# jltsiren/bwt-merge

Measured on AMD Instinct MI355X. Metric: merged Gbases/sec (input1+input2), bit-exact native BWT; value = inputs and result resident in HBM, host_to_host_value = SURVEY 8(d)'s T (page-locked host to page-locked host), higher is better.
Workload: dtype u64

## Files before the change

bwt-merge_amd/csrc/api/context.hip.h:

```cpp
#pragma once


namespace
{

thread_local std::string g_error;

int fail(int code, const char* fmt, ...)
{
  char buf[512];
  va_list ap; va_start(ap, fmt); vsnprintf(buf, sizeof(buf), fmt, ap); va_end(ap);
  g_error = buf;
  return code;
}

inline u64 div_up(u64 a, u64 b) { return (a + b - 1) / b; }

}


struct bwtm_context
{
  int device = -1;
  hipStream_t stream = nullptr;
// ... 3 lines not shown
  std::atomic<long long> live_handles{0};

  bool profiling = false;
  std::string profile_only;
  bool profile_open = false;
  struct Pending { const char* name; hipEvent_t start, stop; };
  std::vector<Pending> pending;
  std::map<std::string, std::pair<double, uint64_t>> totals;
  std::vector<const char*> order;

  std::multimap<u64, void*> free_blocks;
  u64 cached_bytes = 0, held_bytes = 0, peak_bytes = 0;
  struct VBlock { u64 bytes = 0; std::vector<hipMemGenericAllocationHandle_t> chunks; hipEvent_t released = nullptr; };
  bool vmm = false;
  std::vector<hipMemGenericAllocationHandle_t> free_chunks;
  std::map<void*, VBlock> vblocks;
  u64 device_total = 0;
  u64 va_fallbacks = 0;

  void* stream_stage[4] = {nullptr, nullptr, nullptr, nullptr};
  u64 stream_stage_cap[4] = {0, 0, 0, 0};
  u64* host_scratch = nullptr;
  u64 scan1_tiles = 0, pull_scan1_tiles = 0;
  u64 step_forms[3] = {0, 0, 0};
  u64 transcode_forms[16] = {};
};

namespace
{

struct Tuning
{
  long long search_algo = 0;
  long long frontier_unfused = 0;
  long long l1_cap = 0;
  long long emit_path = 0;
  long long round_emits = 1ll << 33;
  long long emit_budget = 0;
  long long frontier_epoch = 512;
  long long eager_cum_budget = 16ll << 30;
  long long upload_chunk = 256ll << 20;
  long long download_chunk = 128ll << 20;
  long long range_ratio = 8;
#ifdef BWTM_EXPERIMENTAL
  long long search_view = 0;
#endif
  long long frontier_stage_out = 1;
  long long frontier_rel = 1;
  long long frontier_parts = 0;
  long long part_capacity = 0;
  long long recs_uniform = 0;
  long long recs_window = 0;
  long long stream_samples_query = 0;
  long long stream_upload = 0;
  long long extract_batch = 1ll << 20;
  long long locate_batch = 1ll << 20;
  long long overlap_batch = 1ll << 20;
  long long mem_batch = 1ll << 20;
  long long approx_batch = 1ll << 16;
  long long correct_batch = 1ll << 20;
  long long ingest_verify = 0;
#ifdef BWTM_DIAGNOSTICS
  long long walk_emit = 0;
  long long walk_blocks = 0;
  long long walk_kernel = 0;
  long long walk_ablate = 0;
// ... 24 lines not shown
void pool_trim(bwtm_context* c);
void stream_stage_free(bwtm_context* c)
{
  for(int k = 0; k < 4; k++) { if(c->stream_stage[k]) { (void)hipHostFree(c->stream_stage[k]); } c->stream_stage[k] = nullptr; c->stream_stage_cap[k] = 0; }
}
void apply_env_tuning();

int context_setup(bwtm_context* c, int device)
{
  int count = 0;
  hipError_t e = hipGetDeviceCount(&count);
  if(e != hipSuccess || count <= 0) { return fail(BWTM_ENODEV, "no HIP device available (%s)", hipGetErrorString(e)); }
  if(device < 0 || device >= count) { return fail(BWTM_EINVAL, "device %d out of range (%d devices)", device, count); }
  HIP_TRY(hipSetDevice(device));
  apply_env_tuning();
  c->device = device;
  HIP_TRY(hipStreamCreateWithFlags(&c->stream, hipStreamNonBlocking));
  HIP_TRY(hipStreamCreateWithFlags(&c->copy_stream, hipStreamNonBlocking));
  HIP_TRY(hipHostMalloc((void**)&c->host_scratch, 128 * sizeof(u64), hipHostMallocDefault));
  vmm_setup(c);
  {
    hipDeviceProp_t prop;
    HIP_TRY(hipGetDeviceProperties(&prop, device));
    int per_cu_scan = 0, per_cu_pull = 0;
    HIP_TRY(hipOccupancyMaxActiveBlocksPerMultiprocessor(&per_cu_scan, (const void*)k_frontier_scan1, BLOCK_THREADS, 0));
    HIP_TRY(hipOccupancyMaxActiveBlocksPerMultiprocessor(&per_cu_pull, (const void*)k_pull_scan1, BLOCK_THREADS, 0));
    c->scan1_tiles = std::min<u64>(FRONTIER_SCAN1_TILES, (u64)std::max(per_cu_scan, 0) * (u64)std::max(prop.multiProcessorCount, 0));
    c->pull_scan1_tiles = std::min<u64>(FRONTIER_SCAN1_TILES, (u64)std::max(per_cu_pull, 0) * (u64)std::max(prop.multiProcessorCount, 0));
  }
  HIP_TRY(hipFuncSetAttribute((const void*)k_part_scatter_sorted, hipFuncAttributeMaxDynamicSharedMemorySize, 96 * 1024));
  HIP_TRY(hipFuncSetAttribute((const void*)k_lf_walk_binned<true>, hipFuncAttributeMaxDynamicSharedMemorySize, 40 * 1024));
#ifdef BWTM_DIAGNOSTICS
  HIP_TRY(hipFuncSetAttribute((const void*)k_lf_walk_lds<true>, hipFuncAttributeMaxDynamicSharedMemorySize, 122 * 1024));
  HIP_TRY(hipFuncSetAttribute((const void*)k_lf_walk_lds<false>, hipFuncAttributeMaxDynamicSharedMemorySize, 82 * 1024));
#endif
  return BWTM_OK;
}

void context_teardown(bwtm_context* c)
{
  if(c->device < 0) { return; }
  (void)hipSetDevice(c->device);
  if(c->stream) { (void)hipStreamSynchronize(c->stream); }
  if(c->copy_stream) { (void)hipStreamSynchronize(c->copy_stream); }
  for(auto& p : c->pending) { (void)hipEventDestroy(p.start); (void)hipEventDestroy(p.stop); }
  c->pending.clear();
  pool_trim(c);
  stream_stage_free(c);
  if(c->host_scratch) { (void)hipHostFree(c->host_scratch); }
  if(c->stream) { (void)hipStreamDestroy(c->stream); }
  if(c->copy_stream) { (void)hipStreamDestroy(c->copy_stream); }
// ... 441 lines not shown
  {
    fail(BWTM_EINVAL, "bwtm_context_destroy: %lld handles of the context are still alive; context not destroyed", context->live_handles.load());
    return;
  }
  context_teardown(context);
  delete context;
}

extern "C" const char* bwtm_last_error(void) { return g_error.c_str(); }

namespace
{
int tune_set(const char* key, long long value)
{
  std::string k(key);
  if(k == "search_algo") { g_tune.search_algo = value; }
  else if(k == "frontier_unfused") { g_tune.frontier_unfused = value; }
  else if(k == "l1_cap") { g_tune.l1_cap = value; }
  else if(k == "emit_path") { g_tune.emit_path = value; }
  else if(k == "round_emits") { g_tune.round_emits = (value > 0 ? value : 1); }
  else if(k == "emit_budget") { g_tune.emit_budget = (value > 0 ? value : 0); }
  else if(k == "frontier_epoch") { g_tune.frontier_epoch = (value > 0 ? value : 512); }
  else if(k == "range_ratio") { g_tune.range_ratio = (value >= 0 ? value : 8); }
#ifdef BWTM_EXPERIMENTAL
  else if(k == "search_view") { g_tune.search_view = (value >= 0 && value <= 2 ? value : 0); }
#endif
  else if(k == "frontier_stage_out") { g_tune.frontier_stage_out = (value != 0); }
  else if(k == "frontier_rel") { g_tune.frontier_rel = (value >= 0 && value <= 2 ? value : 1); }
  else if(k == "frontier_parts") { g_tune.frontier_parts = (value > 0 ? value : 0); }
  else if(k == "stream_samples_query") { g_tune.stream_samples_query = (value != 0); }
  else if(k == "stream_upload") { g_tune.stream_upload = (value != 0); }
  else if(k == "ingest_verify") { g_tune.ingest_verify = (value != 0); }
  else if(k == "extract_batch") { g_tune.extract_batch = (value > 0 ? value : (1ll << 20)); }
  else if(k == "locate_batch") { g_tune.locate_batch = (value > 0 ? std::min<long long>(value, 1ll << 28) : (1ll << 20)); }
  else if(k == "overlap_batch") { g_tune.overlap_batch = (value > 0 ? std::min<long long>(value, 1ll << 28) : (1ll << 20)); }
  else if(k == "mem_batch") { g_tune.mem_batch = (value > 0 ? std::min<long long>(value, 1ll << 28) : (1ll << 20)); }
  else if(k == "approx_batch") { g_tune.approx_batch = (value > 0 ? std::min<long long>(value, 1ll << 28) : (1ll << 16)); }
  else if(k == "correct_batch") { g_tune.correct_batch = (value > 0 ? std::min<long long>(value, 1ll << 28) : (1ll << 20)); }
  else if(k == "part_capacity") { g_tune.part_capacity = value; }
  else if(k == "recs_uniform") { g_tune.recs_uniform = (value > 0 ? 1 : (value < 0 ? -1 : 0)); }
  else if(k == "recs_window") { g_tune.recs_window = (value == 8192 || value == 16384 || value == 32768 ? value : 0); }
  else if(k == "eager_cum_budget") { g_tune.eager_cum_budget = (value > 0 ? value : (16ll << 30)); }
  else if(k == "upload_chunk") { g_tune.upload_chunk = (value > 0 ? value : (256ll << 20)); }
  else if(k == "download_chunk") { g_tune.download_chunk = (value > 0 ? value : (128ll << 20)); }
#ifdef BWTM_DIAGNOSTICS
  else if(k == "walk_emit") { g_tune.walk_emit = value; }
// ... 167 lines not shown
```

bwt-merge_amd/csrc/api/partition.hip.h:

```cpp
#pragma once

extern "C" int bwtm_fslice_set_cuts(bwtm_fslice* fs, const uint64_t* r_cuts, int parts)
{
  if(!fs || !r_cuts || parts < 1 || parts > BWTM_X_MAX_PARTS) { return fail(BWTM_EINVAL, "bwtm_fslice_set_cuts: bad argument (at most %d parts)", BWTM_X_MAX_PARTS); }
  for(int k = 0; k < parts; k++) { if(r_cuts[k] > r_cuts[k + 1] && k + 1 < parts) { return fail(BWTM_EINVAL, "bwtm_fslice_set_cuts: cuts must not decrease"); } }
  if(r_cuts[0] != 0) { return fail(BWTM_EINVAL, "bwtm_fslice_set_cuts: the first cut is 0"); }
  ENTER(fs->ctx);
  if((u32)(5 * parts) > fs->max_pieces) { return fail(BWTM_EINVAL, "bwtm_fslice_set_cuts: more parts than the slice was created for"); }
  fs->ncuts = (u32)parts + 1;
  TRY(fs->cuts.alloc(fs->ncuts * sizeof(u64))); TRY(fs->below.alloc(5ull * fs->ncuts * sizeof(u64), true));
  if(!fs->host_below) { HIP_TRY(hipHostMalloc((void**)&fs->host_below, 5ull * (BWTM_X_MAX_PARTS + 1) * sizeof(u64), hipHostMallocDefault)); }
  if(!fs->dense_lo)
  {
    const u64 fcap = fs->nbl * FR_BLOCK;
    TRY(fslice_export_alloc(fs, fs->dense_lo, fcap));
    if(fs->wide) { TRY(fslice_export_alloc(fs, fs->dense_hi, fcap)); }
    TRY(fs->dense_pieces.alloc((u64)fs->max_pieces * sizeof(DensePiece)));
    HIP_TRY(hipHostMalloc((void**)&fs->host_dense_pieces, (u64)fs->max_pieces * sizeof(DensePiece), hipHostMallocDefault));
  }
  std::memset(fs->host_below, 0, 5ull * (BWTM_X_MAX_PARTS + 1) * sizeof(u64));
  u64 host_cuts[BWTM_X_MAX_PARTS + 1];
  for(int k = 0; k <= parts; k++) { host_cuts[k] = (k == parts ? ~0ull : r_cuts[k]); }
  HIP_TRY(hipMemcpyAsync(fs->cuts.p, host_cuts, fs->ncuts * sizeof(u64), hipMemcpyHostToDevice, CTX.stream));
  HIP_TRY(hipStreamSynchronize(CTX.stream));
// ... 213 lines not shown

extern "C" int bwtm_fslice_nodes_expand(bwtm_fslice* fs)
{
  if(!fs) { return fail(BWTM_EINVAL, "bwtm_fslice_nodes_expand: null argument"); }
  ENTER(fs->ctx);
  if(!fs->node_sp[0]) { return fail(BWTM_EINVAL, "bwtm_fslice_nodes_expand: call bwtm_fslice_nodes_begin first"); }
  const u64 N = fs->nodes;
  u64 alive = 0;
  DevBuf offsets;
  if(N > 0)
  {
    TRY(offsets.alloc((N + 1) * sizeof(u64)));
    HIP_TRY(hipMemcpyAsync(offsets.p, fs->node_cnt[0], N * sizeof(u64), hipMemcpyDeviceToDevice, CTX.stream));
    HIP_TRY(hipMemsetAsync(offsets.as<u64>() + N, 0, sizeof(u64), CTX.stream));
    TRY(device_scan<0>(offsets.as<u64>(), offsets.as<u64>(), N + 1));
    TRY(fetch_u64(offsets.as<u64>() + N, 0));
    HIP_TRY(hipStreamSynchronize(CTX.stream));
    alive = CTX.host_scratch[0];
  }
  if(alive > fs->cap) { return fail(BWTM_EINVAL, "bwtm_fslice_nodes_expand: the nodes stand for %llu sequences, capacity %llu", (unsigned long long)alive, (unsigned long long)fs->cap); }
  fs->nb_out = std::max<u64>(1, div_up(alive, (u64)FR_BLOCK));
  if(N > 0)
  {
    LAUNCH("range_expand", k_range_expand, div_up(N, BLOCK_THREADS), BLOCK_THREADS, (const u64*)fs->node_sp[0], (const u64*)fs->node_r[0], (const u64*)fs->node_cnt[0],
      offsets.as<const u64>(), N, fs->lo_out, fs->hi_out, fs->node_pieces.as<RangePiece>(), fs->node_npieces.as<u32>(), fs->node_piece_cap);
    LAUNCH("range_expand_pieces", k_range_expand_pieces, 2048, BLOCK_THREADS, fs->node_pieces.as<const RangePiece>(), fs->node_npieces.as<const u32>(), fs->node_piece_cap, fs->lo_out, fs->hi_out);
    HIP_TRY(hipMemsetAsync(fs->node_npieces.p, 0, sizeof(u32), CTX.stream));
  }
  LAUNCH("frontier_init", k_frontier_init_tables, div_up(5 * fs->nb_out + 1, BLOCK_THREADS), BLOCK_THREADS, fs->seg_len_out.as<u64>(), fs->seg_phys_out, fs->nb_out, alive);
  fs->nodes = 0;
  TRY(fslice_scan_outputs(fs));
  return BWTM_OK;
}

extern "C" int bwtm_x_index_upload_window(const uint8_t* data, uint64_t nbytes, uint64_t first_position, const uint64_t counts_before[6],
  uint64_t bases, uint64_t sequences, const uint64_t C[7], bwtm_index** out)
{
  ENTER(nullptr);
  return index_upload_window(data, nbytes, first_position, counts_before, bases, sequences, C, false, out);
}

extern "C" int bwtm_x_ra_create_range(const bwtm_index* a, const bwtm_index* b, uint64_t pos_first, uint64_t pos_last, bwtm_ra** out)
{
  return bwtm_ra_create_range(a, b, pos_first, pos_last, out);
}

extern "C" int bwtm_x_ra_or_range(bwtm_ra* dst, const bwtm_ra* src, uint64_t pos_first, uint64_t pos_last)
// ... 52 lines not shown
```

bwt-merge_amd/csrc/api/pmerge.hip.h:

```cpp
#pragma once


namespace
{

int index_upload_window(const u8* data, u64 nbytes, u64 first_position, const u64 counts_before[6], u64 bases, u64 sequences, const u64 C[7], bool on_device, bwtm_index** out)
{
  if(!out || (nbytes > 0 && !data) || !counts_before || !C) { return fail(BWTM_EINVAL, "bwtm_index_upload_window: null argument"); }
  if(nbytes == 0 && bases != 0) { return fail(BWTM_EINVAL, "bwtm_index_upload_window: no bytes of an index of %llu positions", (unsigned long long)bases); }
  u64 before = 0; for(int c = 0; c < 6; c++) { before += counts_before[c]; }
  if(before != first_position || first_position > bases) { return fail(BWTM_EINVAL, "bwtm_index_upload_window: the counts before the bytes add up to %llu, their first position is %llu", (unsigned long long)before, (unsigned long long)first_position); }
  if(on_device && ((uintptr_t)data & 15) != 0) { return fail(BWTM_EINVAL, "bwtm_index_upload_window: a device share must be 16-byte aligned (whole 64-byte blocks of a 16-byte aligned stream)"); }
  bwtm_index* x = new bwtm_index();
  x->ctx = t_ctx; x->nbytes = nbytes;
  auto body = [&]() -> int
  {
    const bool borrow = on_device && nbytes > 0;
    if(borrow) { x->borrowed = data; }
    else { TRY(alloc_native(x->data, nbytes)); }
    int rc = upload_queue(x, (borrow || nbytes == 0) ? nullptr : data);
    if(rc == BWTM_OK) { rc = upload_scan(x, 0); }
    hipError_t e1 = hipStreamSynchronize(CTX.copy_stream), e2 = hipStreamSynchronize(CTX.stream);
    if(rc != BWTM_OK) { return rc; }
    if(e1 != hipSuccess || e2 != hipSuccess) { return fail(BWTM_ENODEV, "upload failed: %s", hipGetErrorString(e1 != hipSuccess ? e1 : e2)); }
// ... 543 lines not shown
    }
    lvl++;
  }
  S.P->info.node_levels = lvl;
  done = (level_nodes == 0);
  nb_out = 1;
  if(done) { return BWTM_OK; }
  TURN(S.G);
  u64 alive = 0;
  if(N > 0)
  {
    TRY(offsets.alloc((N + 1) * 8));
    HIP_TRY(hipMemcpyAsync(offsets.p, cnt.p, N * 8, hipMemcpyDeviceToDevice, CTX.stream));
    HIP_TRY(hipMemsetAsync(offsets.as<u64>() + N, 0, 8, CTX.stream));
    TRY(device_scan<0>(offsets.as<u64>(), offsets.as<u64>(), N + 1));
    TRY(fetch_u64(offsets.as<u64>() + N, 0));
    HIP_TRY(hipStreamSynchronize(CTX.stream));
    alive = CTX.host_scratch[0];
  }
  if(alive > S.cap) { return fail(BWTM_ENOMEM, "bwtm_part_search: the nodes of part %d stand for %llu sequences, capacity %llu", S.g, (unsigned long long)alive, (unsigned long long)S.cap); }
  nb_out = std::max<u64>(1, div_up(alive, (u64)FR_BLOCK));
  if(N > 0)
  {
    LAUNCH("range_expand", k_range_expand, div_up(N, BLOCK_THREADS), BLOCK_THREADS, sp.as<const u64>(), r.as<const u64>(), cnt.as<const u64>(), offsets.as<const u64>(), N,
      S.mine<uint2>(S.lay.lo[0]), (S.wide ? S.mine<unsigned short>(S.lay.hi[0]) : nullptr), pieces.as<RangePiece>(), npieces.as<u32>(), piece_cap);
    LAUNCH("range_expand_pieces", k_range_expand_pieces, 2048, BLOCK_THREADS, pieces.as<const RangePiece>(), npieces.as<const u32>(), piece_cap,
      S.mine<uint2>(S.lay.lo[0]), (S.wide ? S.mine<unsigned short>(S.lay.hi[0]) : nullptr));
  }
  LAUNCH("frontier_init", k_frontier_init_tables, div_up(5 * nb_out + 1, BLOCK_THREADS), BLOCK_THREADS, S.mine<u64>(S.lay.seg_len[0]), S.mine<u64>(S.lay.seg_phys[0]), nb_out, alive);
  return BWTM_OK;
}

int part_search(PartSearch& S)
{
  bwtm_part* P = S.P;
  const u64 m = P->mb;
  const u64 root_first = std::min<u64>(P->cut_b[S.g], m), root_last = std::min<u64>(P->cut_b[S.g + 1], m);
  int owners = 0;
  for(int h = 0; h < S.parts; h++) { if(std::min<u64>(P->cut_b[h + 1], m) > std::min<u64>(P->cut_b[h], m)) { owners++; } }
  const u64 limit = (g_tune.range_ratio > 0 ? std::max<u64>(1, std::min<u64>(m / (u64)g_tune.range_ratio, 1ull << 24)) : 0);
  const bool use_nodes = (limit >= 1 && owners == 1);
  TRY(search_setup(S, use_nodes));
  u64 nb_out = 1;
  int par = 0;
  if(use_nodes)
  {
    bool done = false;
// ... 238 lines not shown
```

bwt-merge_amd/csrc/api/search.hip.h:

```cpp
#pragma once

struct bwtm_ra
{
  bwtm_context* ctx = nullptr;
  bwtm_ra() : ctx(t_ctx) { if(ctx) { ctx->live_handles++; } }
  ~bwtm_ra() { if(ctx) { ctx->live_handles--; } }
  bwtm_ra(const bwtm_ra&) = delete; bwtm_ra& operator=(const bwtm_ra&) = delete;
  u64 na = 0, nb = 0, n_out = 0;
  u64 nrecs_out = 0, nchunks = 0;
  DevBuf owned_bits;
  void* bits_ptr = nullptr;
  template<class T> T* bits_as() const { return (T*)bits_ptr; }
  DevBuf chunk_base;
  bool finalized = false;
  u64 values = 0;
  bool ranged = false;
  u64 range_first = 0, range_last = 0;
  DevBuf range_rel;
  DevBuf super_boff;
  bool windowed = false;
  u64 win_word_first = 0, win_words = 0;
};

#define WHOLE_RA(ra, who) if((ra)->windowed) { return fail(BWTM_EINVAL, who ": a window of a rank array (bwtm_ra_create_range) only serves the merge over partitioned records and the output-range entry points"); }
// ... 171 lines not shown
    {
      LAUNCH_LDS("lf_walk", k_lf_walk_binned<false>, blocks, WB_THREADS, 0, a->view(), b->view(), r_first, r_count, sink, (u32)a->nsup, (u32)b->nsup);
    }

    TRY(partition_level2(l1, gcount, cap, nsub, 1, ra));
  }
  return BWTM_OK;
}

int frontier_flush(bwtm_ra* ra, DevBuf& emit16, u64 emit_cap, DevBuf& emit_base, DevBuf& bound, u64 ntiles, u64 nsteps, u64 tile_first = 0)
{
  if(nsteps == 0) { return BWTM_OK; }
  const u64 nsegs = div_up(ntiles, BOUND_SEG);
  DevBuf segmin; TRY(segmin.alloc(nsteps * nsegs * sizeof(u32)));
  LAUNCH2D("bound_seg_min", k_bound_seg_min, nsegs, nsteps, BLOCK_THREADS, bound.as<const u32>(), ntiles, nsegs, segmin.as<u32>());
  LAUNCH2D("bound_suffix_min", k_bound_suffix_min, nsegs, nsteps, BLOCK_THREADS, bound.as<u32>(), ntiles, nsegs, segmin.as<const u32>(), emit_base.as<const u64>());
  LAUNCH("tile_build", k_tile_build_frontier, ntiles, BLOCK_THREADS, emit16.as<const unsigned short>(), emit_base.as<const u64>(), emit_cap, bound.as<const u32>(),
    ntiles, nsteps, ra->bits_as<u64>() + (tile_first << (TILE_SHIFT - 6)), ra->nchunks * CHUNK_WORDS - (tile_first << (TILE_SHIFT - 6)));
  return BWTM_OK;
}

struct RangeLevels
{
  DevBuf sp[2], r[2], cnt[2], flags, pieces, npieces;
  u64 N = 0, alive = 0, levels = 0;
  u32 piece_cap = 0;
  int cur = 0;
  void release() { for(int k = 0; k < 2; k++) { sp[k].release(); r[k].release(); cnt[k].release(); } flags.release(); pieces.release(); npieces.release(); }
};

int range_phase(const bwtm_index* a, const bwtm_index* b, u64 seq_first, u64 count, bwtm_ra* ra, u64 limit, RangeLevels& L)
{
  const u64 cap = std::min<u64>(5 * limit, count) + 1;
  for(int k = 0; k < 2; k++) { TRY(L.sp[k].alloc(cap * sizeof(u64))); TRY(L.r[k].alloc(cap * sizeof(u64))); TRY(L.cnt[k].alloc(cap * sizeof(u64))); }
  TRY(L.flags.alloc((5 * limit + 1) * sizeof(u64)));
  L.piece_cap = (u32)std::min<u64>(count / 16 + 1024, 1ull << 24);
  TRY(L.pieces.alloc((u64)L.piece_cap * sizeof(RangePiece)));
  TRY(L.npieces.alloc(sizeof(u32), true));
  LAUNCH("range_init", k_range_init, 1, BLOCK_THREADS, L.sp[0].as<u64>(), L.r[0].as<u64>(), L.cnt[0].as<u64>(), seq_first, count, a->m);
  L.N = 1; L.alive = count; L.cur = 0; L.levels = 0;
  while(L.N > 0 && L.N <= limit)
  {
    const int c = L.cur;
    const u64 N = L.N, grid = div_up(N, BLOCK_THREADS);
    LAUNCH("range_step", k_range_step<false>, grid, BLOCK_THREADS, a->view(), b->view(), L.sp[c].as<const u64>(), L.r[c].as<const u64>(), L.cnt[c].as<const u64>(), N,
      L.flags.as<u64>(), (const u64*)nullptr, (u64*)nullptr, (u64*)nullptr, (u64*)nullptr, ra->bits_as<u32>(), L.pieces.as<RangePiece>(), L.npieces.as<u32>(), L.piece_cap);
    LAUNCH("range_emit", k_range_emit, 2048, BLOCK_THREADS, L.pieces.as<const RangePiece>(), L.npieces.as<const u32>(), L.piece_cap, ra->bits_as<u32>());
    HIP_TRY(hipMemsetAsync(L.npieces.p, 0, sizeof(u32), CTX.stream));
    TRY(device_scan<0>(L.flags.as<u64>(), L.flags.as<u64>(), 5 * N + 1));
    LAUNCH("range_children", k_range_step<true>, grid, BLOCK_THREADS, a->view(), b->view(), L.sp[c].as<const u64>(), L.r[c].as<const u64>(), L.cnt[c].as<const u64>(), N,
      (u64*)nullptr, L.flags.as<const u64>(), L.sp[1 - c].as<u64>(), L.r[1 - c].as<u64>(), L.cnt[1 - c].as<u64>(), (u32*)nullptr, (RangePiece*)nullptr, (u32*)nullptr, 0u);
    TRY(fetch_u64(L.flags.as<u64>() + 5 * N, 0));
    HIP_TRY(hipStreamSynchronize(CTX.stream));
    L.N = CTX.host_scratch[0];
    L.cur = 1 - c; L.levels++;
  }
  return BWTM_OK;
}

int range_alive(RangeLevels& L, DevBuf& offsets)
{
  TRY(offsets.alloc((L.N + 1) * sizeof(u64)));
  HIP_TRY(hipMemcpyAsync(offsets.p, L.cnt[L.cur].p, L.N * sizeof(u64), hipMemcpyDeviceToDevice, CTX.stream));
  HIP_TRY(hipMemsetAsync(offsets.as<u64>() + L.N, 0, sizeof(u64), CTX.stream));
  TRY(device_scan<0>(offsets.as<u64>(), offsets.as<u64>(), L.N + 1));
  TRY(fetch_u64(offsets.as<u64>() + L.N, 0));
  HIP_TRY(hipStreamSynchronize(CTX.stream));
  L.alive = CTX.host_scratch[0];
  return BWTM_OK;
}

int range_expand(RangeLevels& L, const DevBuf& offsets, uint2* lo, unsigned short* hi)
{
  const int c = L.cur;
  LAUNCH("range_expand", k_range_expand, div_up(L.N, BLOCK_THREADS), BLOCK_THREADS, L.sp[c].as<const u64>(), L.r[c].as<const u64>(), L.cnt[c].as<const u64>(),
    offsets.as<const u64>(), L.N, lo, hi, L.pieces.as<RangePiece>(), L.npieces.as<u32>(), L.piece_cap);
  LAUNCH("range_expand_pieces", k_range_expand_pieces, 2048, BLOCK_THREADS, L.pieces.as<const RangePiece>(), L.npieces.as<const u32>(), L.piece_cap, lo, hi);
  return BWTM_OK;
}

constexpr u64 FRONTIER_MIN_SEQUENCES = 1ull << 21;

int search_frontier(const bwtm_index* a, const bwtm_index* b, u64 seq_first, u64 count, bwtm_ra* ra)
{
  if(a->n >= (1ull << 40) || b->n >= (1ull << 40) || count >= (1ull << 32)) { return search_partitioned(a, b, seq_first, count, ra); }
  RangeLevels levels;
  DevBuf node_offsets;
  const bool node_phase = (g_tune.range_ratio > 0);
  if(node_phase)
  {
    const u64 limit = std::max<u64>(1, std::min<u64>(count / (u64)g_tune.range_ratio, 1ull << 24));
    TRY(range_phase(a, b, seq_first, count, ra, limit, levels));
    if(levels.N == 0) { return BWTM_OK; }
    TRY(range_alive(levels, node_offsets));
    count = levels.alive;
    if(count == 0) { return BWTM_OK; }
  }
  const u64 ntiles = div_up(ra->n_out + 1, 1ull << TILE_SHIFT);
// ... 363 lines not shown
```

bwt-merge_amd/csrc/kernels/search_range.hip.h:

```cpp
#pragma once

constexpr u32 RANGE_INLINE_WORDS = 4;
constexpr u32 RANGE_PIECE_WORDS = 2048;
constexpr u32 RANGE_EXPAND_INLINE = 48;
constexpr u32 RANGE_EXPAND_PIECE = 1024;

struct RangePiece { u64 first; u64 count; u64 aux; u64 dst; };

__device__ inline void range_set_bits(u32* bits, u64 p0, u64 p1)
{
  for(u64 w = p0 >> 5; w <= ((p1 - 1) >> 5); w++)
  {
    const u64 lo = (w << 5 > p0 ? w << 5 : p0), hi = (((w + 1) << 5) < p1 ? (w + 1) << 5 : p1);
    const u32 n = (u32)(hi - lo), sh = (u32)(lo & 31);
    const u32 mask = (n == 32 ? 0xFFFFFFFFu : ((1u << n) - 1u) << sh);
    atomicOr(bits + w, mask);
  }
}

__global__ void __launch_bounds__(BLOCK_THREADS) k_range_init(u64* sp, u64* r, u64* cnt, u64 seq_first, u64 count, u64 m_a)
{
  if(blockIdx.x == 0 && threadIdx.x == 0) { sp[0] = seq_first; r[0] = m_a; cnt[0] = count; }
}

template<bool WRITE>
__global__ void __launch_bounds__(BLOCK_THREADS) k_range_step(IndexView A, IndexView B, const u64* sp, const u64* r, const u64* cnt, u64 N,
  u64* flags, const u64* prefix, u64* sp_next, u64* r_next, u64* cnt_next, u32* bits, RangePiece* pieces, u32* npieces, u32 piece_cap)
{
  const u64 u = (u64)blockIdx.x * BLOCK_THREADS + threadIdx.x;
  if(u >= N) { return; }
  const u64 s = sp[u], k = cnt[u], rr = r[u];
  u64 rs[6], re[6];
  index_ranks(B, s, rs);
  index_ranks(B, s + k, re);
  if(!WRITE)
  {
#pragma unroll
    for(u32 c = 1; c < 6; c++) { flags[(u64)(c - 1) * N + u] = (re[c] > rs[c] ? 1 : 0); }
    if(u == 0) { flags[5 * N] = 0; }
    const u64 p0 = s + rr, p1 = p0 + k;
    if(((p1 - 1) >> 5) - (p0 >> 5) < RANGE_INLINE_WORDS) { range_set_bits(bits, p0, p1); }
    else
    {
      const u64 per = (u64)RANGE_PIECE_WORDS * 32;
      const u64 first_cut = ((p0 / per) + 1) * per;
      const u32 n = (u32)(p1 <= first_cut ? 1 : 1 + (p1 - first_cut + per - 1) / per);
      const u32 at = atomicAdd(npieces, n);
      u64 b = p0;
      for(u32 q = 0; q < n; q++)
      {
        u64 e = (b / per + 1) * per; if(e > p1) { e = p1; }
        if(at + q < piece_cap) { RangePiece pc; pc.first = b; pc.count = e - b; pc.aux = 0; pc.dst = 0; pieces[at + q] = pc; }
        else { range_set_bits(bits, b, e); }
        b = e;
      }
    }
  }
  else
  {
    u64 ra[6];
    index_ranks(A, rr, ra);
#pragma unroll
    for(u32 c = 1; c < 6; c++)
    {
      if(re[c] > rs[c])
      {
        const u64 d = prefix[(u64)(c - 1) * N + u];
        sp_next[d] = B.C[c] + rs[c];
        cnt_next[d] = re[c] - rs[c];
        r_next[d] = A.C[c] + ra[c];
      }
    }
  }
}

__global__ void __launch_bounds__(BLOCK_THREADS) k_range_emit(const RangePiece* pieces, const u32* npieces, u32 piece_cap, u32* bits)
{
  u32 n = *npieces; if(n > piece_cap) { n = piece_cap; }
  for(u32 q = blockIdx.x; q < n; q += gridDim.x)
  {
    const u64 p0 = pieces[q].first, p1 = p0 + pieces[q].count;
    const u64 w0 = p0 >> 5, w1 = (p1 - 1) >> 5;
    for(u64 w = w0 + threadIdx.x; w <= w1; w += BLOCK_THREADS)
    {
      const u64 lo = (w << 5 > p0 ? w << 5 : p0), hi = (((w + 1) << 5) < p1 ? (w + 1) << 5 : p1);
      const u32 nb = (u32)(hi - lo), sh = (u32)(lo & 31);
      atomicOr(bits + w, (nb == 32 ? 0xFFFFFFFFu : ((1u << nb) - 1u) << sh));
    }
  }
}

__device__ inline void range_store_element(uint2* lo, unsigned short* hi, u64 g, u64 i, u64 r)
{
  lo[g] = make_uint2((u32)i, (u32)r);
  if(hi) { hi[g] = (unsigned short)(((i >> 32) & 0xFF) | (((r >> 32) & 0xFF) << 8)); }
}

__global__ void __launch_bounds__(BLOCK_THREADS) k_range_expand(const u64* sp, const u64* r, const u64* cnt, const u64* offset, u64 N,
  uint2* lo, unsigned short* hi, RangePiece* pieces, u32* npieces, u32 piece_cap)
{
  const u64 u = (u64)blockIdx.x * BLOCK_THREADS + threadIdx.x;
  if(u >= N) { return; }
  const u64 s = sp[u], k = cnt[u], rr = r[u], g0 = offset[u];
  if(k <= RANGE_EXPAND_INLINE) { for(u64 j = 0; j < k; j++) { range_store_element(lo, hi, g0 + j, s + j, rr); } return; }
  const u32 n = (u32)((k + RANGE_EXPAND_PIECE - 1) / RANGE_EXPAND_PIECE);
  const u32 at = atomicAdd(npieces, n);
  for(u32 q = 0; q < n; q++)
  {
    const u64 b = (u64)q * RANGE_EXPAND_PIECE;
    const u64 c = (k - b < (u64)RANGE_EXPAND_PIECE ? k - b : (u64)RANGE_EXPAND_PIECE);
    if(at + q < piece_cap) { RangePiece pc; pc.first = s + b; pc.count = c; pc.aux = rr; pc.dst = g0 + b; pieces[at + q] = pc; }
    else { for(u64 j = 0; j < c; j++) { range_store_element(lo, hi, g0 + b + j, s + b + j, rr); } }
  }
}

__global__ void __launch_bounds__(BLOCK_THREADS) k_range_expand_pieces(const RangePiece* pieces, const u32* npieces, u32 piece_cap, uint2* lo, unsigned short* hi)
{
  u32 n = *npieces; if(n > piece_cap) { n = piece_cap; }
  for(u32 q = blockIdx.x; q < n; q += gridDim.x)
  {
    const RangePiece pc = pieces[q];
    for(u64 j = threadIdx.x; j < pc.count; j += BLOCK_THREADS) { range_store_element(lo, hi, pc.dst + j, pc.first + j, pc.aux); }
  }
}

__global__ void __launch_bounds__(BLOCK_THREADS) k_frontier_init_tables(u64* seg_len, u64* seg_phys, u64 nb_max, u64 count)
// ... 12 lines not shown
```

Measured before the change: 93.29.

## Fuse range-search level into single-pass kernel with decoupled look-back scan

Replaces the per-level two-kernel flow (flag pass, device scan, children pass) with one persistent kernel that computes child counts, publishes tile aggregates and inclusive prefixes, and scatters children in one pass using decoupled look-back. Children are written into five class-strided segments, so a RangeForm mapping is threaded through the counts and expand kernels. This removes two kernel launches and a full device scan per level, plus the flag buffer traffic. In exchange it adds spin-polling with a timeout that falls back to a compaction and a two-pass redo, tag-based tile reuse, and dependence on forward progress across co-resident blocks.

Result: no change. 94.20 (median of 6 runs) (+1.0%).

```diff
diff --git a/bwt-merge_amd/csrc/api/context.hip.h b/bwt-merge_amd/csrc/api/context.hip.h
--- a/bwt-merge_amd/csrc/api/context.hip.h
+++ b/bwt-merge_amd/csrc/api/context.hip.h
@@ -49,6 +49,7 @@
   u64 stream_stage_cap[4] = {0, 0, 0, 0};
   u64* host_scratch = nullptr;
   u64 scan1_tiles = 0, pull_scan1_tiles = 0;
+  u64 range_grid = 0;
   u64 step_forms[3] = {0, 0, 0};
   u64 transcode_forms[16] = {};
 };
@@ -69,6 +70,10 @@
   long long upload_chunk = 256ll << 20;
   long long download_chunk = 128ll << 20;
   long long range_ratio = 8;
+  long long range_single_pass = 1;
+  long long range_grid = 0;
+  long long range_piece_cap = 0;
+  long long range_expire_level = 0;
 #ifdef BWTM_EXPERIMENTAL
   long long search_view = 0;
 #endif
@@ -139,11 +144,13 @@
   {
     hipDeviceProp_t prop;
     HIP_TRY(hipGetDeviceProperties(&prop, device));
-    int per_cu_scan = 0, per_cu_pull = 0;
+    int per_cu_scan = 0, per_cu_pull = 0, per_cu_range = 0;
     HIP_TRY(hipOccupancyMaxActiveBlocksPerMultiprocessor(&per_cu_scan, (const void*)k_frontier_scan1, BLOCK_THREADS, 0));
     HIP_TRY(hipOccupancyMaxActiveBlocksPerMultiprocessor(&per_cu_pull, (const void*)k_pull_scan1, BLOCK_THREADS, 0));
     c->scan1_tiles = std::min<u64>(FRONTIER_SCAN1_TILES, (u64)std::max(per_cu_scan, 0) * (u64)std::max(prop.multiProcessorCount, 0));
     c->pull_scan1_tiles = std::min<u64>(FRONTIER_SCAN1_TILES, (u64)std::max(per_cu_pull, 0) * (u64)std::max(prop.multiProcessorCount, 0));
+    HIP_TRY(hipOccupancyMaxActiveBlocksPerMultiprocessor(&per_cu_range, (const void*)k_range_level, BLOCK_THREADS, 0));
+    c->range_grid = (u64)std::max(per_cu_range, 0) * (u64)std::max(prop.multiProcessorCount, 0);
   }
   HIP_TRY(hipFuncSetAttribute((const void*)k_part_scatter_sorted, hipFuncAttributeMaxDynamicSharedMemorySize, 96 * 1024));
   HIP_TRY(hipFuncSetAttribute((const void*)k_lf_walk_binned<true>, hipFuncAttributeMaxDynamicSharedMemorySize, 40 * 1024));
@@ -631,6 +638,10 @@
   else if(k == "emit_budget") { g_tune.emit_budget = (value > 0 ? value : 0); }
   else if(k == "frontier_epoch") { g_tune.frontier_epoch = (value > 0 ? value : 512); }
   else if(k == "range_ratio") { g_tune.range_ratio = (value >= 0 ? value : 8); }
+  else if(k == "range_single_pass") { g_tune.range_single_pass = (value == 0 ? 0 : 1); }
+  else if(k == "range_grid") { g_tune.range_grid = (value > 0 ? value : 0); }
+  else if(k == "range_piece_cap") { g_tune.range_piece_cap = (value > 0 ? std::min<long long>(value, 1ll << 24) : 0); }
+  else if(k == "range_expire_level") { g_tune.range_expire_level = (value > 0 ? value : 0); }
 #ifdef BWTM_EXPERIMENTAL
   else if(k == "search_view") { g_tune.search_view = (value >= 0 && value <= 2 ? value : 0); }
 #endif
diff --git a/bwt-merge_amd/csrc/api/partition.hip.h b/bwt-merge_amd/csrc/api/partition.hip.h
--- a/bwt-merge_amd/csrc/api/partition.hip.h
+++ b/bwt-merge_amd/csrc/api/partition.hip.h
@@ -259,7 +259,7 @@
   fs->nb_out = std::max<u64>(1, div_up(alive, (u64)FR_BLOCK));
   if(N > 0)
   {
-    LAUNCH("range_expand", k_range_expand, div_up(N, BLOCK_THREADS), BLOCK_THREADS, (const u64*)fs->node_sp[0], (const u64*)fs->node_r[0], (const u64*)fs->node_cnt[0],
+    LAUNCH("range_expand", k_range_expand, div_up(N, BLOCK_THREADS), BLOCK_THREADS, (const u64*)fs->node_sp[0], (const u64*)fs->node_r[0], (const u64*)fs->node_cnt[0], range_dense(N),
       offsets.as<const u64>(), N, fs->lo_out, fs->hi_out, fs->node_pieces.as<RangePiece>(), fs->node_npieces.as<u32>(), fs->node_piece_cap);
     LAUNCH("range_expand_pieces", k_range_expand_pieces, 2048, BLOCK_THREADS, fs->node_pieces.as<const RangePiece>(), fs->node_npieces.as<const u32>(), fs->node_piece_cap, fs->lo_out, fs->hi_out);
     HIP_TRY(hipMemsetAsync(fs->node_npieces.p, 0, sizeof(u32), CTX.stream));
diff --git a/bwt-merge_amd/csrc/api/pmerge.hip.h b/bwt-merge_amd/csrc/api/pmerge.hip.h
--- a/bwt-merge_amd/csrc/api/pmerge.hip.h
+++ b/bwt-merge_amd/csrc/api/pmerge.hip.h
@@ -589,7 +589,7 @@
   nb_out = std::max<u64>(1, div_up(alive, (u64)FR_BLOCK));
   if(N > 0)
   {
-    LAUNCH("range_expand", k_range_expand, div_up(N, BLOCK_THREADS), BLOCK_THREADS, sp.as<const u64>(), r.as<const u64>(), cnt.as<const u64>(), offsets.as<const u64>(), N,
+    LAUNCH("range_expand", k_range_expand, div_up(N, BLOCK_THREADS), BLOCK_THREADS, sp.as<const u64>(), r.as<const u64>(), cnt.as<const u64>(), range_dense(N), offsets.as<const u64>(), N,
       S.mine<uint2>(S.lay.lo[0]), (S.wide ? S.mine<unsigned short>(S.lay.hi[0]) : nullptr), pieces.as<RangePiece>(), npieces.as<u32>(), piece_cap);
     LAUNCH("range_expand_pieces", k_range_expand_pieces, 2048, BLOCK_THREADS, pieces.as<const RangePiece>(), npieces.as<const u32>(), piece_cap,
       S.mine<uint2>(S.lay.lo[0]), (S.wide ? S.mine<unsigned short>(S.lay.hi[0]) : nullptr));
diff --git a/bwt-merge_amd/csrc/api/search.hip.h b/bwt-merge_amd/csrc/api/search.hip.h
--- a/bwt-merge_amd/csrc/api/search.hip.h
+++ b/bwt-merge_amd/csrc/api/search.hip.h
@@ -217,38 +217,92 @@
 
 struct RangeLevels
 {
-  DevBuf sp[2], r[2], cnt[2], flags, pieces, npieces;
-  u64 N = 0, alive = 0, levels = 0;
-  u32 piece_cap = 0;
+  DevBuf sp[2], r[2], cnt[2], flags, pieces, npieces, tiles, out;
+  u64 N = 0, alive = 0, levels = 0, limit = 0;
+  RangeForm form;
+  u32 piece_cap = 0, tag = 0;
   int cur = 0;
-  void release() { for(int k = 0; k < 2; k++) { sp[k].release(); r[k].release(); cnt[k].release(); } flags.release(); pieces.release(); npieces.release(); }
+  void release()
+  {
+    for(int k = 0; k < 2; k++) { sp[k].release(); r[k].release(); cnt[k].release(); }
+    flags.release(); pieces.release(); npieces.release(); tiles.release(); out.release();
+  }
 };
 
+RangeForm range_dense(u64 N) { RangeForm f; f.first[0] = 0; for(int c = 1; c < 5; c++) { f.first[c] = N; } f.stride = N; return f; }
+
+int range_level_two_pass(const bwtm_index* a, const bwtm_index* b, bwtm_ra* ra, RangeLevels& L, int c, const char* first_label)
+{
+  const u64 N = L.N, grid = div_up(N, BLOCK_THREADS);
+  if(!L.flags.p) { TRY(L.flags.alloc((5 * L.limit + 1) * sizeof(u64))); }
+  LAUNCH(first_label, k_range_step<false>, grid, BLOCK_THREADS, a->view(), b->view(), L.sp[c].as<const u64>(), L.r[c].as<const u64>(), L.cnt[c].as<const u64>(), N,
+    L.flags.as<u64>(), (const u64*)nullptr, (u64*)nullptr, (u64*)nullptr, (u64*)nullptr, ra->bits_as<u32>(), L.pieces.as<RangePiece>(), L.npieces.as<u32>(), L.piece_cap);
+  LAUNCH("range_emit", k_range_emit, 2048, BLOCK_THREADS, L.pieces.as<const RangePiece>(), L.npieces.as<const u32>(), L.piece_cap, ra->bits_as<u32>());
+  HIP_TRY(hipMemsetAsync(L.npieces.p, 0, sizeof(u32), CTX.stream));
+  TRY(device_scan<0>(L.flags.as<u64>(), L.flags.as<u64>(), 5 * N + 1));
+  LAUNCH("range_children", k_range_step<true>, grid, BLOCK_THREADS, a->view(), b->view(), L.sp[c].as<const u64>(), L.r[c].as<const u64>(), L.cnt[c].as<const u64>(), N,
+    (u64*)nullptr, L.flags.as<const u64>(), L.sp[1 - c].as<u64>(), L.r[1 - c].as<u64>(), L.cnt[1 - c].as<u64>(), (u32*)nullptr, (RangePiece*)nullptr, (u32*)nullptr, 0u);
+  TRY(fetch_u64(L.flags.as<u64>() + 5 * N, 0));
+  return BWTM_OK;
+}
+
 int range_phase(const bwtm_index* a, const bwtm_index* b, u64 seq_first, u64 count, bwtm_ra* ra, u64 limit, RangeLevels& L)
 {
-  const u64 cap = std::min<u64>(5 * limit, count) + 1;
+  const bool single = (g_tune.range_single_pass != 0 && CTX.range_grid > 0);
+  const u64 cap = (single ? 5 * limit : std::min<u64>(5 * limit, count)) + 1;
   for(int k = 0; k < 2; k++) { TRY(L.sp[k].alloc(cap * sizeof(u64))); TRY(L.r[k].alloc(cap * sizeof(u64))); TRY(L.cnt[k].alloc(cap * sizeof(u64))); }
-  TRY(L.flags.alloc((5 * limit + 1) * sizeof(u64)));
   L.piece_cap = (u32)std::min<u64>(count / 16 + 1024, 1ull << 24);
+  if(g_tune.range_piece_cap > 0) { L.piece_cap = (u32)g_tune.range_piece_cap; }
   TRY(L.pieces.alloc((u64)L.piece_cap * sizeof(RangePiece)));
   TRY(L.npieces.alloc(sizeof(u32), true));
+  const u64 tile_bytes = div_up(limit, BLOCK_THREADS) * 4 * sizeof(u64);
+  if(single) { TRY(L.tiles.alloc(tile_bytes, true)); TRY(L.out.alloc(8 * sizeof(u64), true)); }
   LAUNCH("range_init", k_range_init, 1, BLOCK_THREADS, L.sp[0].as<u64>(), L.r[0].as<u64>(), L.cnt[0].as<u64>(), seq_first, count, a->m);
-  L.N = 1; L.alive = count; L.cur = 0; L.levels = 0;
+  L.N = 1; L.alive = count; L.cur = 0; L.levels = 0; L.limit = limit; L.tag = 0; L.form = range_dense(1);
   while(L.N > 0 && L.N <= limit)
   {
     const int c = L.cur;
-    const u64 N = L.N, grid = div_up(N, BLOCK_THREADS);
-    LAUNCH("range_step", k_range_step<false>, grid, BLOCK_THREADS, a->view(), b->view(), L.sp[c].as<const u64>(), L.r[c].as<const u64>(), L.cnt[c].as<const u64>(), N,
-      L.flags.as<u64>(), (const u64*)nullptr, (u64*)nullptr, (u64*)nullptr, (u64*)nullptr, ra->bits_as<u32>(), L.pieces.as<RangePiece>(), L.npieces.as<u32>(), L.piece_cap);
+    const u64 N = L.N;
+    if(!single)
+    {
+      TRY(range_level_two_pass(a, b, ra, L, c, "range_step"));
+      HIP_TRY(hipStreamSynchronize(CTX.stream));
+      L.N = CTX.host_scratch[0]; L.form = range_dense(L.N);
+      L.cur = 1 - c; L.levels++;
+      continue;
+    }
+    u64 grid = std::min<u64>(div_up(N, BLOCK_THREADS), CTX.range_grid);
+    if(g_tune.range_grid > 0) { grid = std::min<u64>(grid, (u64)g_tune.range_grid); }
+    if(++L.tag >= (1u << RANGE_TAG_BITS)) { HIP_TRY(hipMemsetAsync(L.tiles.p, 0, tile_bytes, CTX.stream)); L.tag = 1; }
+    const u32 budget = ((u64)g_tune.range_expire_level == L.levels + 1 ? 0u : RANGE_POLL_BUDGET);
+    LAUNCH("range_step", k_range_level, grid, BLOCK_THREADS, a->view(), b->view(), L.sp[c].as<const u64>(), L.r[c].as<const u64>(), L.cnt[c].as<const u64>(), L.form, N,
+      L.sp[1 - c].as<u64>(), L.r[1 - c].as<u64>(), L.cnt[1 - c].as<u64>(), ra->bits_as<u32>(), L.pieces.as<RangePiece>(), L.npieces.as<u32>(), L.piece_cap,
+      L.tiles.as<unsigned long long>(), L.tag, budget, L.out.as<unsigned long long>());
     LAUNCH("range_emit", k_range_emit, 2048, BLOCK_THREADS, L.pieces.as<const RangePiece>(), L.npieces.as<const u32>(), L.piece_cap, ra->bits_as<u32>());
     HIP_TRY(hipMemsetAsync(L.npieces.p, 0, sizeof(u32), CTX.stream));
-    TRY(device_scan<0>(L.flags.as<u64>(), L.flags.as<u64>(), 5 * N + 1));
-    LAUNCH("range_children", k_range_step<true>, grid, BLOCK_THREADS, a->view(), b->view(), L.sp[c].as<const u64>(), L.r[c].as<const u64>(), L.cnt[c].as<const u64>(), N,
-      (u64*)nullptr, L.flags.as<const u64>(), L.sp[1 - c].as<u64>(), L.r[1 - c].as<u64>(), L.cnt[1 - c].as<u64>(), (u32*)nullptr, (RangePiece*)nullptr, (u32*)nullptr, 0u);
-    TRY(fetch_u64(L.flags.as<u64>() + 5 * N, 0));
+    TRY(fetch_u64(L.out.as<u64>(), 0, 7));
     HIP_TRY(hipStreamSynchronize(CTX.stream));
-    L.N = CTX.host_scratch[0];
-    L.cur = 1 - c; L.levels++;
+    if(CTX.host_scratch[6] == 0)
+    {
+      L.form.first[0] = 0; L.form.stride = N;
+      for(int k = 1; k < 5; k++) { L.form.first[k] = L.form.first[k - 1] + CTX.host_scratch[k - 1]; }
+      L.N = CTX.host_scratch[5];
+      L.cur = 1 - c; L.levels++;
+      continue;
+    }
+    HIP_TRY(hipMemsetAsync(L.out.p, 0, 8 * sizeof(u64), CTX.stream));
+    for(int k = 0; k < 5; k++)
+    {
+      const u64 n = (k < 4 ? L.form.first[k + 1] : N) - L.form.first[k], src = (u64)k * L.form.stride, dst = L.form.first[k];
+      if(n == 0) { continue; }
+      HIP_TRY(hipMemcpyAsync(L.sp[1 - c].as<u64>() + dst, L.sp[c].as<u64>() + src, n * sizeof(u64), hipMemcpyDeviceToDevice, CTX.stream));
+      HIP_TRY(hipMemcpyAsync(L.r[1 - c].as<u64>() + dst, L.r[c].as<u64>() + src, n * sizeof(u64), hipMemcpyDeviceToDevice, CTX.stream));
+      HIP_TRY(hipMemcpyAsync(L.cnt[1 - c].as<u64>() + dst, L.cnt[c].as<u64>() + src, n * sizeof(u64), hipMemcpyDeviceToDevice, CTX.stream));
+    }
+    TRY(range_level_two_pass(a, b, ra, L, 1 - c, "range_redo"));
+    HIP_TRY(hipStreamSynchronize(CTX.stream));
+    L.N = CTX.host_scratch[0]; L.form = range_dense(L.N);
+    L.levels++;
   }
   return BWTM_OK;
 }
@@ -256,8 +310,7 @@
 int range_alive(RangeLevels& L, DevBuf& offsets)
 {
   TRY(offsets.alloc((L.N + 1) * sizeof(u64)));
-  HIP_TRY(hipMemcpyAsync(offsets.p, L.cnt[L.cur].p, L.N * sizeof(u64), hipMemcpyDeviceToDevice, CTX.stream));
-  HIP_TRY(hipMemsetAsync(offsets.as<u64>() + L.N, 0, sizeof(u64), CTX.stream));
+  LAUNCH("range_counts", k_range_counts, div_up(L.N + 1, BLOCK_THREADS), BLOCK_THREADS, L.cnt[L.cur].as<const u64>(), L.form, L.N, offsets.as<u64>());
   TRY(device_scan<0>(offsets.as<u64>(), offsets.as<u64>(), L.N + 1));
   TRY(fetch_u64(offsets.as<u64>() + L.N, 0));
   HIP_TRY(hipStreamSynchronize(CTX.stream));
@@ -268,7 +321,7 @@
 int range_expand(RangeLevels& L, const DevBuf& offsets, uint2* lo, unsigned short* hi)
 {
   const int c = L.cur;
-  LAUNCH("range_expand", k_range_expand, div_up(L.N, BLOCK_THREADS), BLOCK_THREADS, L.sp[c].as<const u64>(), L.r[c].as<const u64>(), L.cnt[c].as<const u64>(),
+  LAUNCH("range_expand", k_range_expand, div_up(L.N, BLOCK_THREADS), BLOCK_THREADS, L.sp[c].as<const u64>(), L.r[c].as<const u64>(), L.cnt[c].as<const u64>(), L.form,
     offsets.as<const u64>(), L.N, lo, hi, L.pieces.as<RangePiece>(), L.npieces.as<u32>(), L.piece_cap);
   LAUNCH("range_expand_pieces", k_range_expand_pieces, 2048, BLOCK_THREADS, L.pieces.as<const RangePiece>(), L.npieces.as<const u32>(), L.piece_cap, lo, hi);
   return BWTM_OK;
diff --git a/bwt-merge_amd/csrc/kernels/search_range.hip.h b/bwt-merge_amd/csrc/kernels/search_range.hip.h
--- a/bwt-merge_amd/csrc/kernels/search_range.hip.h
+++ b/bwt-merge_amd/csrc/kernels/search_range.hip.h
@@ -7,6 +7,18 @@
 
 struct RangePiece { u64 first; u64 count; u64 aux; u64 dst; };
 
+struct RangeForm { u64 first[5]; u64 stride; };
+
+__device__ inline u64 range_phys(const RangeForm& f, u64 u)
+{
+  u64 c = 0, base = 0;
+  if(u >= f.first[1]) { c = 1; base = f.first[1]; }
+  if(u >= f.first[2]) { c = 2; base = f.first[2]; }
+  if(u >= f.first[3]) { c = 3; base = f.first[3]; }
+  if(u >= f.first[4]) { c = 4; base = f.first[4]; }
+  return c * f.stride + (u - base);
+}
+
 __device__ inline void range_set_bits(u32* bits, u64 p0, u64 p1)
 {
   for(u64 w = p0 >> 5; w <= ((p1 - 1) >> 5); w++)
@@ -15,6 +27,23 @@
     const u32 n = (u32)(hi - lo), sh = (u32)(lo & 31);
     const u32 mask = (n == 32 ? 0xFFFFFFFFu : ((1u << n) - 1u) << sh);
     atomicOr(bits + w, mask);
+  }
+}
+
+__device__ inline void range_set_run(u32* bits, u64 p0, u64 p1, RangePiece* pieces, u32* npieces, u32 piece_cap)
+{
+  if(((p1 - 1) >> 5) - (p0 >> 5) < RANGE_INLINE_WORDS) { range_set_bits(bits, p0, p1); return; }
+  const u64 per = (u64)RANGE_PIECE_WORDS * 32;
+  const u64 first_cut = ((p0 / per) + 1) * per;
+  const u32 n = (u32)(p1 <= first_cut ? 1 : 1 + (p1 - first_cut + per - 1) / per);
+  const u32 at = atomicAdd(npieces, n);
+  u64 b = p0;
+  for(u32 q = 0; q < n; q++)
+  {
+    u64 e = (b / per + 1) * per; if(e > p1) { e = p1; }
+    if(at + q < piece_cap) { RangePiece pc; pc.first = b; pc.count = e - b; pc.aux = 0; pc.dst = 0; pieces[at + q] = pc; }
+    else { range_set_bits(bits, b, e); }
+    b = e;
   }
 }
 
@@ -38,23 +67,7 @@
 #pragma unroll
     for(u32 c = 1; c < 6; c++) { flags[(u64)(c - 1) * N + u] = (re[c] > rs[c] ? 1 : 0); }
     if(u == 0) { flags[5 * N] = 0; }
-    const u64 p0 = s + rr, p1 = p0 + k;
-    if(((p1 - 1) >> 5) - (p0 >> 5) < RANGE_INLINE_WORDS) { range_set_bits(bits, p0, p1); }
-    else
-    {
-      const u64 per = (u64)RANGE_PIECE_WORDS * 32;
-      const u64 first_cut = ((p0 / per) + 1) * per;
-      const u32 n = (u32)(p1 <= first_cut ? 1 : 1 + (p1 - first_cut + per - 1) / per);
-      const u32 at = atomicAdd(npieces, n);
-      u64 b = p0;
-      for(u32 q = 0; q < n; q++)
-      {
-        u64 e = (b / per + 1) * per; if(e > p1) { e = p1; }
-        if(at + q < piece_cap) { RangePiece pc; pc.first = b; pc.count = e - b; pc.aux = 0; pc.dst = 0; pieces[at + q] = pc; }
-        else { range_set_bits(bits, b, e); }
-        b = e;
-      }
-    }
+    range_set_run(bits, s + rr, s + rr + k, pieces, npieces, piece_cap);
   }
   else
   {
@@ -74,6 +87,146 @@
   }
 }
 
+constexpr u32 RANGE_TAG_BITS = 14;
+constexpr u32 RANGE_POLL_BUDGET = 1u << 18;
+
+__device__ inline u32 range_word_tag(unsigned long long w) { return (u32)(w >> 50); }
+
+__global__ void __launch_bounds__(BLOCK_THREADS) __attribute__((amdgpu_waves_per_eu(4, 4))) k_range_level(IndexView A, IndexView B, const u64* sp, const u64* r, const u64* cnt, RangeForm form, u64 N,
+  u64* sp_next, u64* r_next, u64* cnt_next, u32* bits, RangePiece* pieces, u32* npieces, u32 piece_cap,
+  unsigned long long* tiles, u32 tag, u32 poll_budget, unsigned long long* out)
+{
+  constexpr u32 NW = BLOCK_THREADS / WAVE;
+  __shared__ u32 wave_count[NW][5];
+  __shared__ u32 tile_before[5];
+  __shared__ u32 stop_in, stop_out;
+  const u32 lane = lane_id(), wave = threadIdx.x >> 6;
+  const u64 ntiles = (N + BLOCK_THREADS - 1) / BLOCK_THREADS;
+  const unsigned long long tagged = (unsigned long long)tag << 50;
+  for(u64 t = blockIdx.x; t < ntiles; t += gridDim.x)
+  {
+    if(threadIdx.x == 0) { stop_in = (u32)__hip_atomic_load(out + 6, __ATOMIC_RELAXED, __HIP_MEMORY_SCOPE_AGENT); }
+    __syncthreads();
+    if(stop_in != 0) { return; }
+    const u64 u = t * BLOCK_THREADS + threadIdx.x;
+    const bool live = (u < N);
+    const u64 at = (live ? range_phys(form, u) : 0);
+    const u64 s = (live ? sp[at] : 0), k = (live ? cnt[at] : 0), rr = (live ? r[at] : 0);
+    u64 rs[6], re[6], ra[6];
+    index_ranks(B, s, rs);
+    index_ranks(B, s + k, re);
+    index_ranks(A, rr, ra);
+    u32 mine[5];
+#pragma unroll
+    for(u32 c = 1; c < 6; c++)
+    {
+      const u64 m = __ballot(re[c] > rs[c]);
+      mine[c - 1] = (u32)__popcll(m & ((1ull << lane) - 1ull));
+      if(lane == 0) { wave_count[wave][c - 1] = (u32)__popcll(m); }
+    }
+    __syncthreads();
+    u32 total[5];
+#pragma unroll
+    for(u32 c = 0; c < 5; c++)
+    {
+      total[c] = 0;
+#pragma unroll
+      for(u32 w = 0; w < NW; w++) { if(w == wave) { mine[c] += total[c]; } total[c] += wave_count[w][c]; }
+    }
+    if(wave == 0)
+    {
+      if(lane == 0)
+      {
+        __hip_atomic_store(tiles + 4 * t, tagged | ((unsigned long long)total[0] << 36) | ((unsigned long long)total[1] << 27) | ((unsigned long long)total[2] << 18) |
+          ((unsigned long long)total[3] << 9) | (unsigned long long)total[4], __ATOMIC_RELAXED, __HIP_MEMORY_SCOPE_AGENT);
+      }
+    }
+    if(live) { range_set_run(bits, s + rr, s + rr + k, pieces, npieces, piece_cap); }
+    if(wave == 0)
+    {
+      u32 before[5] = {0, 0, 0, 0, 0};
+      bool expired = (poll_budget == 0);
+      u32 polls = 0;
+      u64 top = t;
+      while(top > 0 && !expired)
+      {
+        u32 v[5] = {0, 0, 0, 0, 0};
+        bool running = (lane >= top), timeout = false;
+        if(!running)
+        {
+          const unsigned long long* w = tiles + 4 * (top - 1 - lane);
+          for(;;)
+          {
+            const unsigned long long p0 = __hip_atomic_load(w + 1, __ATOMIC_RELAXED, __HIP_MEMORY_SCOPE_AGENT);
+            const unsigned long long p1 = __hip_atomic_load(w + 2, __ATOMIC_RELAXED, __HIP_MEMORY_SCOPE_AGENT);
+            const unsigned long long p2 = __hip_atomic_load(w + 3, __ATOMIC_RELAXED, __HIP_MEMORY_SCOPE_AGENT);
+            if(range_word_tag(p0) == tag && range_word_tag(p1) == tag && range_word_tag(p2) == tag)
+            {
+              v[0] = (u32)(p0 >> 25) & 0x1FFFFFFu; v[1] = (u32)p0 & 0x1FFFFFFu; v[2] = (u32)(p1 >> 25) & 0x1FFFFFFu; v[3] = (u32)p1 & 0x1FFFFFFu; v[4] = (u32)p2 & 0x1FFFFFFu;
+              running = true; break;
+            }
+            const unsigned long long a = __hip_atomic_load(w, __ATOMIC_RELAXED, __HIP_MEMORY_SCOPE_AGENT);
+            if(range_word_tag(a) == tag)
+            {
+              v[0] = (u32)(a >> 36) & 0x1FFu; v[1] = (u32)(a >> 27) & 0x1FFu; v[2] = (u32)(a >> 18) & 0x1FFu; v[3] = (u32)(a >> 9) & 0x1FFu; v[4] = (u32)a & 0x1FFu;
+              break;
+            }
+            if(polls >= poll_budget) { timeout = true; break; }
+            polls++;
+            __builtin_amdgcn_s_sleep(1);
+          }
+        }
+        if(__ballot(timeout) != 0) { expired = true; break; }
+        const u64 have = __ballot(running);
+        const u32 first = (have != 0 ? (u32)__builtin_ctzll(have) : (u32)WAVE);
+#pragma unroll
+        for(u32 c = 0; c < 5; c++) { before[c] += (u32)__builtin_amdgcn_readlane((int)wave_incl_sum32(lane <= first ? v[c] : 0u), WAVE - 1); }
+        top = (first < (u32)WAVE ? 0 : top - WAVE);
+      }
+      if(lane == 0)
+      {
+        stop_out = (expired ? 1u : 0u);
+        if(expired) { __hip_atomic_store(out + 6, 1ull, __ATOMIC_RELAXED, __HIP_MEMORY_SCOPE_AGENT); }
+        else
+        {
+          unsigned long long incl[5];
+#pragma unroll
+          for(u32 c = 0; c < 5; c++) { tile_before[c] = before[c]; incl[c] = (unsigned long long)(before[c] + total[c]); }
+          __hip_atomic_store(tiles + 4 * t + 1, tagged | (incl[0] << 25) | incl[1], __ATOMIC_RELAXED, __HIP_MEMORY_SCOPE_AGENT);
+          __hip_atomic_store(tiles + 4 * t + 2, tagged | (incl[2] << 25) | incl[3], __ATOMIC_RELAXED, __HIP_MEMORY_SCOPE_AGENT);
+          __hip_atomic_store(tiles + 4 * t + 3, tagged | incl[4], __ATOMIC_RELAXED, __HIP_MEMORY_SCOPE_AGENT);
+          if(t + 1 == ntiles)
+          {
+#pragma unroll
+            for(u32 c = 0; c < 5; c++) { out[c] = incl[c]; }
+            out[5] = incl[0] + incl[1] + incl[2] + incl[3] + incl[4];
+          }
+        }
+      }
+    }
+    __syncthreads();
+    if(stop_out != 0) { return; }
+#pragma unroll
+    for(u32 c = 1; c < 6; c++)
+    {
+      if(re[c] > rs[c])
+      {
+        const u64 d = (u64)(c - 1) * N + tile_before[c - 1] + mine[c - 1];
+        sp_next[d] = B.C[c] + rs[c];
+        cnt_next[d] = re[c] - rs[c];
+        r_next[d] = A.C[c] + ra[c];
+      }
+    }
+  }
+}
+
+__global__ void __launch_bounds__(BLOCK_THREADS) k_range_counts(const u64* cnt, RangeForm form, u64 N, u64* out)
+{
+  const u64 u = (u64)blockIdx.x * BLOCK_THREADS + threadIdx.x;
+  if(u < N) { out[u] = cnt[range_phys(form, u)]; }
+  if(u == N) { out[u] = 0; }
+}
+
 __global__ void __launch_bounds__(BLOCK_THREADS) k_range_emit(const RangePiece* pieces, const u32* npieces, u32 piece_cap, u32* bits)
 {
   u32 n = *npieces; if(n > piece_cap) { n = piece_cap; }
@@ -96,12 +249,13 @@
   if(hi) { hi[g] = (unsigned short)(((i >> 32) & 0xFF) | (((r >> 32) & 0xFF) << 8)); }
 }
 
-__global__ void __launch_bounds__(BLOCK_THREADS) k_range_expand(const u64* sp, const u64* r, const u64* cnt, const u64* offset, u64 N,
+__global__ void __launch_bounds__(BLOCK_THREADS) k_range_expand(const u64* sp, const u64* r, const u64* cnt, RangeForm form, const u64* offset, u64 N,
   uint2* lo, unsigned short* hi, RangePiece* pieces, u32* npieces, u32 piece_cap)
 {
   const u64 u = (u64)blockIdx.x * BLOCK_THREADS + threadIdx.x;
   if(u >= N) { return; }
-  const u64 s = sp[u], k = cnt[u], rr = r[u], g0 = offset[u];
+  const u64 phys = range_phys(form, u);
+  const u64 s = sp[phys], k = cnt[phys], rr = r[phys], g0 = offset[u];
   if(k <= RANGE_EXPAND_INLINE) { for(u64 j = 0; j < k; j++) { range_store_element(lo, hi, g0 + j, s + j, rr); } return; }
   const u32 n = (u32)((k + RANGE_EXPAND_PIECE - 1) / RANGE_EXPAND_PIECE);
   const u32 at = atomicAdd(npieces, n);
```
